# Lymphatus/caesium-clt

Hardware: AMD Instinct MI355X
Metric: megapixels/sec JPEG q=80 1920x1080 batch (higher is better)
Workload: dtype int32

## Files before the change

### caesium-clt_amd/csrc/k_trellis.hip

```cpp
#include <algorithm>
#include <atomic>
#include <cassert>
#include <utility>

#include "kernels.h"

namespace csh {

#define CSH_TR_CAP 16
#define CSH_TR_WGU uint32_t(CSH_TR_WG)
#define CSH_TR_SPILL (63 - CSH_TR_CAP)
#define CSH_TR_MAXWG 2048
size_t trellis_spill_words(uint32_t nslots) { return size_t(nslots) * CSH_TR_SPILL * 3u * CSH_TR_WGU; }

#ifdef CSH_EMUL
#define CSH_ANY(p) (p)
#define CSH_WAVE_OR(v) (v)
#define CSH_SPILL_LD(ptr) (*(ptr))
#define CSH_SPILL_ST(ptr, v) (*(ptr) = (v))
#else
#define CSH_ANY(p) (__ballot(p) != 0ull)
__device__ __forceinline__ static unsigned tr_wave_or(unsigned v) {
    const unsigned n = 32u - unsigned(__clz(v));
    unsigned r = 0;
    if (__ballot(n >= 8u)) r = 8u;
    if (__ballot(n >= r + 4u)) r += 4u;
    if (__ballot(n >= r + 2u)) r += 2u;
    if (__ballot(n >= r + 1u)) r += 1u;
    return r ? 1u << (r - 1u) : 0u;
}
#define CSH_WAVE_OR(v) tr_wave_or(v)
#define CSH_SPILL_LD(ptr) __builtin_nontemporal_load(ptr)
#define CSH_SPILL_ST(ptr, v) __builtin_nontemporal_store((v), (ptr))
#endif

using Oct8 = std::integer_sequence<int, 0, 1, 2, 3, 4, 5, 6, 7>;
static constexpr uint8_t kN2Z[64] = {0,  1,  5,  6,  14, 15, 27, 28, 2,  4,  7,  13, 16, 26, 29, 42, 3,  8,  12, 17, 25, 30,
                                     41, 43, 9,  11, 18, 24, 31, 40, 44, 53, 10, 19, 23, 32, 39, 45, 52, 54, 20, 22, 33, 38,
                                     46, 51, 55, 60, 21, 34, 37, 47, 50, 56, 59, 61, 35, 36, 48, 49, 57, 58, 62, 63};
template <int I>
__device__ __forceinline__ static int tr_half(const uint4 &v) {
    uint32_t w = (I / 2 == 0) ? v.x : (I / 2 == 1) ? v.y : (I / 2 == 2) ? v.z : v.w;
    return (I & 1) ? (int(w) >> 16) : (int(w << 16) >> 16);
}
template <int J, int... I>
__device__ __forceinline__ static void tr_unpack(int r[64], const uint4 &v, std::integer_sequence<int, I...>) { ((r[8 * J + I] = tr_half<I>(v)), ...); }
template <int... J>
__device__ __forceinline__ static void tr_load(const int16_t *__restrict__ blk, int r[64], std::integer_sequence<int, J...>) {
    const uint4 v[8] = {*reinterpret_cast<const uint4 *>(blk + CSH_RAW_OCT * J)...};
    (tr_unpack<J>(r, v[J], Oct8()), ...);
}
__device__ __forceinline__ static int tr_level(int x, int d, uint32_t mul, uint32_t sh) {
    const uint32_t a = uint32_t(x + (d >> 1)) << sh;
    return int(uint32_t((uint64_t(a & 0xFFFFFFu) * uint64_t(mul & 0xFFFFFFu)) >> 32));
}
__device__ __forceinline__ static int tr_bitlen(unsigned v) { return 32 - __clz(v); }
__device__ __forceinline__ static float tr_bits_f(uint32_t u) { float f; memcpy(&f, &u, 4); return f; }
__device__ __forceinline__ static uint32_t tr_f_bits(float f) { uint32_t u; memcpy(&u, &f, 4); return u; }

#define TRELLIS_LAMBDA_C1 0x1.ae89f995ad3adp+14
#define TRELLIS_LAMBDA_C2 0x1.6a09e667f3bcdp+16
#define TRELLIS_MAX_LEVEL 1023

struct TrLds {
    float (*A)[CSH_TR_WG];
    float (*Z)[CSH_TR_WG];
    uint32_t (*P)[CSH_TR_WG];
    const float *lenf;
    const float *runf;
    int lenEOB;
    const int32_t *q8;
    const uint32_t *qmul, *qsh;
    const float *lt;
    const float *rcp;
};

__device__ __forceinline__ static void trellis_stage(const TrellisCtx &c, uint32_t wi, float *s_lenf, float *s_runf, int *s_eob, int32_t *s_q8, uint32_t *s_qmul, uint32_t *s_qsh, float *s_lt, float *s_rcp) {
    const TrellisWork &w = c.work[wi];
    const ImgDesc &im = c.imgs[w.image];
    const DevQuant &Q = c.quant[im.qt_out[w.comp]];
    const int tid = int(threadIdx.x);
    const uint8_t *size = c.tables[w.table_ac].size;
    for (int i = tid; i < 16 * 11; i += CSH_TR_WG) {
        const int r = i / 11, sz = i % 11 + 1, l = sz <= 10 ? size[(r << 4) | sz] : 0;
        s_lenf[i] = l ? float(l + sz) : 1e38f;
    }
    if (tid < 4) s_runf[tid] = tid == 0 ? 0.0f : (size[0xF0] ? float(tid * int(size[0xF0])) : 1e38f);
    if (tid == 0) *s_eob = size[0x00];
    if (tid < 64) { s_q8[tid] = Q.div[tid]; s_qmul[tid] = Q.mul[tid]; s_qsh[tid] = Q.sh[tid]; s_lt[tid] = Q.lt[tid]; s_rcp[tid] = Q.rcp[tid]; }
}

__device__ __forceinline__ static void trellis_block(const TrellisCtx &c, uint32_t wi, uint32_t j, uint32_t wg_slot, const TrLds &L) {
    const TrellisWork &w = c.work[wi];
    const ImgDesc &im = c.imgs[w.image];
    const CompGeom g = im.out[w.comp];
    const int tid = int(threadIdx.x);
    const uint32_t slot = j * CSH_TR_WGU + uint32_t(tid);
    if (slot >= w.nunits) return;
    const uint32_t u = c.perm ? c.perm[w.unit_base + slot] : slot;
    const int by = int(u) / g.real_bw, b = by * g.bw + (int(u) - by * g.real_bw);
    uint32_t *sp = c.spill + size_t(wg_slot) * (CSH_TR_SPILL * 3u * CSH_TR_WGU) + uint32_t(tid);

    int r[64];
    tr_load(c.raw + raw_index(g.tile_base - c.raw_tile0, b), r, Oct8());
    CSH_SCHED_FENCE();
    float norm = 0.0f;
    CSH_UNROLL
    for (int n = 1; n < 64; n++) { const float vf = float(r[kN2Z[n]]); norm = norm + vf * vf; }
    norm = float(double(norm) / 63.0);
    const float lambda = float(TRELLIS_LAMBDA_C1 / (TRELLIS_LAMBDA_C2 + double(norm)));
    c.dcrec[w.unit_base + u] = (uint64_t(tr_f_bits(lambda)) << 32) | (uint32_t(r[0]) & 0xFFFFu);
    CSH_SCHED_FENCE();
    if (c.debug & 1u) return;

    uint32_t ne = 0;
    float Zrun = 0.0f;
    CSH_UNROLL
    for (int k = 1; k < 64; k++) {
        const int v = r[k], x = v < 0 ? -v : v;
        const float xf = float(x);
        int qv = int(tr_f_bits(__builtin_fmaf(xf, L.rcp[k], 12582912.0f)) & 0xFFFFu);
        qv = qv > TRELLIS_MAX_LEVEL ? TRELLIS_MAX_LEVEL : qv;
        if (qv) {
            const uint32_t P = uint32_t(x) | (uint32_t(k) << 15) | (uint32_t(qv) << 21) | (v < 0 ? 0x80000000u : 0u);
            if (ne < CSH_TR_CAP) { L.Z[ne][tid] = Zrun; L.P[ne][tid] = P; }
            else { CSH_SPILL_ST(sp + ((ne - CSH_TR_CAP) * 3u + 1u) * CSH_TR_WGU, tr_f_bits(Zrun)); CSH_SPILL_ST(sp + ((ne - CSH_TR_CAP) * 3u + 2u) * CSH_TR_WGU, P); }
            ne++;
        }
        Zrun = ((xf * xf) * lambda) * L.lt[k] + Zrun;
    }
    const float Z63 = Zrun;
    CSH_SCHED_FENCE();

    const float lenEOBf = float(L.lenEOB);
    if (c.debug & 2u) ne = 0;
    for (uint32_t t = 0; CSH_ANY(t < ne); t++) {
        const bool on = t < ne;
        float Zp; uint32_t P;
        if (t < CSH_TR_CAP) { Zp = L.Z[t][tid]; P = L.P[t][tid]; }
        else { Zp = tr_bits_f(CSH_SPILL_LD(sp + ((t - CSH_TR_CAP) * 3u + 1u) * CSH_TR_WGU)); P = CSH_SPILL_LD(sp + ((t - CSH_TR_CAP) * 3u + 2u) * CSH_TR_WGU); }
        if (!on) { Zp = 0.0f; P = 0u; }
        const int x = int(P & 0x7FFFu), kpos = int((P >> 15) & 63u), qval = int((P >> 21) & 1023u);
        const int q8 = L.q8[kpos];
        const float ltk = L.lt[kpos];
        const int ncand = on ? tr_bitlen(unsigned(qval)) : 0;
        const int ncmax = tr_bitlen(CSH_WAVE_OR(on ? unsigned(qval) : 0u));
        float dist[10];
        CSH_UNROLL
        for (int kc = 0; kc < 10; kc++) {
            dist[kc] = 1e38f;
            if (kc >= ncmax) continue;
            const int cand = kc < ncand - 1 ? (2 << kc) - 1 : qval;
            const int delta = __mul24(cand, q8) - x;
            dist[kc] = kc < ncand ? (float(__mul24(delta, delta)) * lambda) * ltk : 1e38f;
        }
        float bestc = 1e38f;
        uint32_t bestsel = 0;
        auto from = [&](int jj, int posj, float Aj, float Zj) {
            const int zr = kpos - 1 - posj;
            const float runf = L.runf[(zr >> 4) & 3];
            const float *lf = L.lenf + 11 * (zr & 15);
            const float tj = (Zp - Zj) + Aj;
            const uint32_t sel0 = uint32_t(jj + 1) << 4;
            CSH_UNROLL
            for (int kc = 0; kc < 10; kc++) {
                if (kc >= ncmax) break;
                const float cost = ((lf[kc] + runf) + dist[kc]) + tj;
                const bool better = cost < bestc;
                bestc = better ? cost : bestc;
                bestsel = better ? (sel0 | uint32_t(kc)) : bestsel;
            }
        };
        from(-1, 0, 0.0f, 0.0f);
        const int t_lds = int(t) < CSH_TR_CAP ? int(t) : CSH_TR_CAP;
        if (ncmax <= 4) {
            auto batch = [&](auto KCV) {
                constexpr int KC = decltype(KCV)::value;
                for (int j0 = 0; j0 < t_lds; j0 += 4) {
                    uint32_t Pj[4]; float Aj[4], Zj[4];
                    CSH_UNROLL
                    for (int i = 0; i < 4; i++) { const int r = j0 + i < CSH_TR_CAP ? j0 + i : CSH_TR_CAP - 1; Pj[i] = L.P[r][tid]; Aj[i] = L.A[r][tid]; Zj[i] = L.Z[r][tid]; }
                    float cost[4][KC];
                    CSH_UNROLL
                    for (int i = 0; i < 4; i++) {
                        const int zr = kpos - 1 - int((Pj[i] >> 15) & 63u);
                        const float runf = L.runf[(zr >> 4) & 3];
                        const float *lf = L.lenf + 11 * (zr & 15);
                        const float tj = j0 + i < t_lds ? (Zp - Zj[i]) + Aj[i] : 1e38f;
                        CSH_UNROLL
                        for (int kc = 0; kc < KC; kc++) cost[i][kc] = ((lf[kc] + runf) + dist[kc]) + tj;
                    }
                    CSH_UNROLL
                    for (int i = 0; i < 4; i++) {
                        CSH_UNROLL
                        for (int kc = 0; kc < KC; kc++) {
                            const bool better = cost[i][kc] < bestc;
                            bestc = better ? cost[i][kc] : bestc;
                            bestsel = better ? ((uint32_t(j0 + i + 1) << 4) | uint32_t(kc)) : bestsel;
                        }
                    }
                }
            };
            if (ncmax <= 1) batch(std::integral_constant<int, 1>());
            else if (ncmax == 2) batch(std::integral_constant<int, 2>());
            else if (ncmax == 3) batch(std::integral_constant<int, 3>());
            else batch(std::integral_constant<int, 4>());
        } else
            for (int jj = 0; jj < t_lds; jj++) from(jj, int((L.P[jj][tid] >> 15) & 63u), L.A[jj][tid], L.Z[jj][tid]);
        for (int jj = CSH_TR_CAP; jj < int(t); jj++) {
            const uint32_t *q = sp + (uint32_t(jj - CSH_TR_CAP) * 3u) * CSH_TR_WGU;
            from(jj, int((CSH_SPILL_LD(q + 2 * CSH_TR_WG) >> 15) & 63u), tr_bits_f(CSH_SPILL_LD(q)), tr_bits_f(CSH_SPILL_LD(q + CSH_TR_WG)));
        }
        if (on) {
            const int bk = int(bestsel & 15u);
            const uint32_t level = uint32_t(bk < ncand - 1 ? (2 << bk) - 1 : qval);
            const float Zi = (float(__mul24(x, x)) * lambda) * ltk + Zp;
            const uint32_t P2 = (bestsel >> 4) | ((level == uint32_t(qval) && qval < TRELLIS_MAX_LEVEL) ? 0x4000u : 0u) | (uint32_t(kpos) << 15) | (level << 21) | (P & 0x80000000u);
            if (t < CSH_TR_CAP) { L.A[t][tid] = bestc; L.Z[t][tid] = Zi; L.P[t][tid] = P2; }
            else { uint32_t *q = sp + ((t - CSH_TR_CAP) * 3u) * CSH_TR_WGU; CSH_SPILL_ST(q, tr_f_bits(bestc)); CSH_SPILL_ST(q + CSH_TR_WG, tr_f_bits(Zi)); CSH_SPILL_ST(q + 2 * CSH_TR_WG, P2); }
        }
    }

    float best = Z63 + lenEOBf;
    int last = -1;
    for (uint32_t e = 0; CSH_ANY(e < ne); e++) {
        float Ae, Ze; uint32_t Pe;
        if (e < CSH_TR_CAP) { Ae = L.A[e][tid]; Ze = L.Z[e][tid]; Pe = L.P[e][tid]; }
        else { const uint32_t *q = sp + ((e - CSH_TR_CAP) * 3u) * CSH_TR_WGU; Ae = tr_bits_f(CSH_SPILL_LD(q)); Ze = tr_bits_f(CSH_SPILL_LD(q + CSH_TR_WG)); Pe = CSH_SPILL_LD(q + 2 * CSH_TR_WG); }
        float cost = (Ae + Z63) - Ze;
        if (int((Pe >> 15) & 63u) < 63) cost = cost + lenEOBf;
        if (e < ne && cost < best) { best = cost; last = int(e); }
    }

    if (c.debug & 4u) return;
    uint64_t kept = 0;
    for (int e = last; CSH_ANY(e >= 0);) {
        if (e >= 0) {
            uint32_t Pe;
            if (e < CSH_TR_CAP) Pe = L.P[e][tid]; else Pe = CSH_SPILL_LD(sp + (uint32_t(e - CSH_TR_CAP) * 3u + 2u) * CSH_TR_WGU);
            kept |= 1ull << e;
            e = int(Pe & 63u) - 1;
        }
    }
    const bool to_tile = !(c.ac_lists && w.ac_lists);
    int16_t *dst = to_tile ? c.coef + coef_index(g.tile_base, b, 0) : nullptr;
    uint32_t *lst = nullptr;
    if (c.nz_pool && w.nzset != 0xFFFFFFFFu) {
        const NzSet &S = c.nzsets[w.nzset];
        const NzList &L0 = c.nzlists[S.list[0]];
        const uint32_t rec = L0.chunk0 + (u >> 8);
        if (c.nz_chunk_cnt[rec]) lst = c.nz_pool + L0.base + c.nz_chunk_off[rec] + c.blk_off[w.unit_base + u];
    }
    uint32_t room = ne;
    if (lst && c.blk_cnt) {
        room = c.blk_cnt[w.unit_base + u];
#ifdef CSH_EMUL
        if (room != ne) { fprintf(stderr, "k_trellis_ac: block %u of unit %u has %u list entries but %u levels\n", u, w.unit_base, room, ne); abort(); }
#endif
    }
    for (uint32_t e0 = 0; CSH_ANY(e0 < ne); e0 += 4) {
        uint32_t ent[4] = {0u, 0u, 0u, 0u};
        CSH_UNROLL
        for (uint32_t i = 0; i < 4; i++) {
            const uint32_t e = e0 + i;
            if (e < ne) {
                uint32_t Pe;
                if (e < CSH_TR_CAP) Pe = L.P[e][tid]; else Pe = CSH_SPILL_LD(sp + ((e - CSH_TR_CAP) * 3u + 2u) * CSH_TR_WGU);
                const int pos = int((Pe >> 15) & 63u), level = ((kept >> e) & 1ull) ? int((Pe >> 21) & 1023u) : 0;
                if (to_tile && !(((kept >> e) & 1ull) && (Pe & 0x4000u))) dst[coef_off(pos)] = int16_t((Pe >> 31) ? -level : level);
                ent[i] = uint32_t(pos) | ((Pe >> 31) ? 128u : 0u) | (uint32_t(level) << 8) | ((u & 255u) << 23);
            }
        }
        if (lst && e0 < ne && e0 < room) {
            if (e0 + 4 <= ne && e0 + 4 <= room) {
#ifdef CSH_EMUL
                memcpy(lst + e0, ent, 16);
#else
                typedef uint32_t tr_u32x4_a4 __attribute__((ext_vector_type(4), aligned(4)));
                tr_u32x4_a4 v; v.x = ent[0]; v.y = ent[1]; v.z = ent[2]; v.w = ent[3];
                *reinterpret_cast<tr_u32x4_a4 *>(lst + e0) = v;
#endif
            } else {
                CSH_UNROLL
                for (uint32_t i = 0; i < 4; i++) if (e0 + i < ne && e0 + i < room) lst[e0 + i] = ent[i];
            }
        }
    }
}

__global__ void __launch_bounds__(256) k_trellis_sort(TrellisCtx c) {
    CSH_SHARED uint32_t s_cnt[64];
    const TrellisWork w = c.work[blockIdx.x];
    const uint8_t *cnt = c.blk_cnt + w.unit_base;
    uint32_t *perm = c.perm + w.unit_base;
    CSH_PHASE_LOOP(4) {
        if (phase == 0) { if (threadIdx.x < 64) s_cnt[threadIdx.x] = 0; continue; }
        if (phase == 1) { for (uint32_t u = threadIdx.x; u < w.nunits; u += 256) atomicAdd(&s_cnt[cnt[u] & 63u], 1u); continue; }
        if (phase == 2) {
            if (threadIdx.x == 0) { uint32_t at = 0; for (int k = 63; k >= 0; k--) { const uint32_t n = s_cnt[k]; s_cnt[k] = at; at += n; } }
            continue;
        }
        for (uint32_t u = threadIdx.x; u < w.nunits; u += 256) perm[atomicAdd(&s_cnt[cnt[u] & 63u], 1u)] = u;
    }
}
void launch_trellis_sort(hipStream_t st, const TrellisCtx &c) { if (c.nwork && c.perm && c.blk_cnt) CSH_LAUNCH_PHASED(k_trellis_sort, 4, dim3(unsigned(c.nwork)), dim3(256), st, c); }

__global__ void __launch_bounds__(CSH_TR_WG) k_trellis_ac(TrellisCtx c) {
    CSH_SHARED float s_A[CSH_TR_CAP][CSH_TR_WG];
    CSH_SHARED float s_Z[CSH_TR_CAP][CSH_TR_WG];
    CSH_SHARED uint32_t s_P[CSH_TR_CAP][CSH_TR_WG];
    CSH_SHARED float s_lenf[16 * 11 + 16];
    CSH_SHARED float s_runf[4];
    CSH_SHARED int s_eob;
    CSH_SHARED int32_t s_q8[64];
    CSH_SHARED uint32_t s_qmul[64];
    CSH_SHARED uint32_t s_qsh[64];
    CSH_SHARED float s_lt[64];
    CSH_SHARED float s_rcp[64];
    TrLds L; L.A = s_A; L.Z = s_Z; L.P = s_P; L.lenf = s_lenf; L.runf = s_runf; L.q8 = s_q8; L.qmul = s_qmul; L.qsh = s_qsh; L.lt = s_lt; L.rcp = s_rcp;
#ifdef CSH_EMUL
    CSH_PHASE_LOOP(2) {
        const TrellisRun rn = c.runs[blockIdx.x];
        if (phase == 0) { trellis_stage(c, rn.work, s_lenf, s_runf, &s_eob, s_q8, s_qmul, s_qsh, s_lt, s_rcp); continue; }
        L.lenEOB = s_eob;
        for (uint32_t j = rn.j; j < rn.j + rn.n; j++) trellis_block(c, rn.work, j, 0u, L);
    }
#else
    CSH_SHARED uint32_t s_run;
    for (;;) {
        if (threadIdx.x == 0) s_run = atomicAdd(c.queue, 1u);
        __syncthreads();
        const uint32_t ri = s_run;
        if (ri >= c.nruns) break;
        const TrellisRun rn = c.runs[ri];
        trellis_stage(c, rn.work, s_lenf, s_runf, &s_eob, s_q8, s_qmul, s_qsh, s_lt, s_rcp);
        __syncthreads();
        L.lenEOB = s_eob;
        for (uint32_t j = rn.j; j < rn.j + rn.n; j++) trellis_block(c, rn.work, j, blockIdx.x, L);
        __syncthreads();
    }
#endif
}

__device__ static const uint8_t kStdDcLen[2][12] = {{2, 3, 3, 3, 3, 3, 4, 5, 6, 7, 8, 9}, {2, 2, 2, 3, 4, 5, 6, 7, 8, 9, 10, 11}};

__global__ void __launch_bounds__(64) k_trellis_dc(TrellisCtx c) {
    const uint32_t ri = blockIdx.x * blockDim.x + threadIdx.x;
    if (ri >= c.nrows) return;
    const uint32_t rr = c.rows[ri];
    const TrellisWork w = c.work[rr >> 16];
    const ImgDesc &im = c.imgs[w.image];
    const CompGeom g = im.out[w.comp];
    const DevQuant &Q = c.quant[im.qt_out[w.comp]];
    const int row = int(rr & 0xFFFFu);
    int ncand = (2 + 60 / int(Q.q[0])) | 1;
    ncand = ncand > 9 ? 9 : ncand;
    CSH_SHARED float s_costs[64][13];
    float *s_cost = s_costs[threadIdx.x & 63u];
    for (int i = 0; i < 12; i++) s_cost[i] = float(i + int(w.table_dc < 0 ? kStdDcLen[w.dc_cls ? 1 : 0][i] : c.tables[w.table_dc].size[i]));
    s_cost[12] = __builtin_inff();
    const int q = Q.div[0];
    const uint32_t qmul = Q.mul[0], qsh = Q.sh[0];
    const float lt0 = Q.lt[0];
    const int half = ncand / 2;
    int last_dc = 0;
    const int by1 = (row + 1) * g.v < g.real_bh ? (row + 1) * g.v : g.real_bh;
    for (int by = row * g.v; by < by1; by++) {
        float acc[9];
        int cprev[9];
        CSH_UNROLL
        for (int k = 0; k < 9; k++) { acc[k] = 0.0f; cprev[k] = 0; }
        int qprev = 0, sprev = 0;
        bool cprev_clamped = false;
        uint64_t rec_next = c.dcrec[w.unit_base + uint32_t(by * g.real_bw)];
        for (int bi = 0; bi < g.real_bw; bi++) {
            const uint32_t u = uint32_t(by * g.real_bw + bi);
            const uint64_t rec = rec_next;
            if (bi + 1 < g.real_bw) rec_next = c.dcrec[w.unit_base + u + 1u];
            const int raw0 = int(int16_t(uint16_t(rec & 0xFFFFu)));
            const float lambda_dc = tr_bits_f(uint32_t(rec >> 32)) * lt0;
            const int x = raw0 < 0 ? -raw0 : raw0;
            const int qval = tr_level(x, q, qmul, qsh);
            const int sgn = raw0 < 0 ? 1 : 0;
            const bool clamped = qval + half > TRELLIS_MAX_LEVEL;
            uint64_t bt = 0;
            float nacc[9];
            int ccur[9];
            float dist[9];
            CSH_UNROLL
            for (int k = 0; k < 9; k++) {
                int cand = qval - half + k;
                cand = cand > TRELLIS_MAX_LEVEL ? TRELLIS_MAX_LEVEL : cand;
                cand = cand < -TRELLIS_MAX_LEVEL ? -TRELLIS_MAX_LEVEL : cand;
                const int delta = k < ncand ? cand * q - x : 0;
                dist[k] = k < ncand ? float(delta * delta) * lambda_dc : __builtin_inff();
                ccur[k] = sgn ? -cand : cand;
            }
            if (bi == 0) {
                CSH_UNROLL
                for (int k = 0; k < 9; k++) { const int d = ccur[k] - last_dc, bits = tr_bitlen(unsigned(d < 0 ? -d : d)); nacc[k] = s_cost[bits] + dist[k]; }
            } else if (clamped || cprev_clamped) {
                CSH_UNROLL
                for (int k = 0; k < 9; k++) {
                    float bc = 0.0f;
                    uint32_t bl = 0;
                    CSH_UNROLL
                    for (int l = 0; l < 9; l++) {
                        const int d = ccur[k] - cprev[l], bits = tr_bitlen(unsigned(d < 0 ? -d : d));
                        const float cost = (s_cost[bits] + dist[k]) + acc[l];
                        if (l == 0 || cost < bc) { bc = cost; bl = uint32_t(l); }
                    }
                    nacc[k] = bc;
                    bt |= uint64_t(bl) << (4 * k);
                }
            } else {
                const bool same = sgn == sprev;
                const int base = same ? qval - qprev : qval + qprev - 2 * half;
                float cd[17];
                CSH_UNROLL
                for (int i = 0; i < 17; i++) { const int d = base + (i - 8); const int dd = same ? d : d + 8; cd[i] = s_cost[tr_bitlen(unsigned(dd < 0 ? -dd : dd))]; }
                CSH_UNROLL
                for (int k = 0; k < 9; k++) {
                    float bc = 0.0f;
                    uint32_t bl = 0;
                    CSH_UNROLL
                    for (int l = 0; l < 9; l++) {
                        const float cbits = same ? cd[k - l + 8] : cd[k + l];
                        const float cost = (cbits + dist[k]) + acc[l];
                        if (l == 0 || cost < bc) { bc = cost; bl = uint32_t(l); }
                    }
                    nacc[k] = bc;
                    bt |= uint64_t(bl) << (4 * k);
                }
            }
            CSH_UNROLL
            for (int k = 0; k < 9; k++) { acc[k] = nacc[k]; cprev[k] = ccur[k]; }
            qprev = qval; sprev = sgn; cprev_clamped = clamped;
            c.dcbt[w.unit_base + u] = bt | (uint64_t(uint32_t(qval)) << 36) | (uint64_t(raw0 < 0 ? 1u : 0u) << 47);
        }
        float bv = acc[0];
        uint32_t j = 0;
        CSH_UNROLL
        for (int i = 1; i < 9; i++) if (i < ncand && acc[i] < bv) { bv = acc[i]; j = uint32_t(i); }
        uint64_t bt_next = c.dcbt[w.unit_base + uint32_t(by * g.real_bw + g.real_bw - 1)];
        for (int bi = g.real_bw - 1; bi >= 0; bi--) {
            const uint64_t rec = bt_next;
            if (bi > 0) bt_next = c.dcbt[w.unit_base + uint32_t(by * g.real_bw + bi - 1)];
            int cand = int((rec >> 36) & 2047u) - half + int(j);
            cand = cand > TRELLIS_MAX_LEVEL ? TRELLIS_MAX_LEVEL : cand;
            cand = cand < -TRELLIS_MAX_LEVEL ? -TRELLIS_MAX_LEVEL : cand;
            cand = ((rec >> 47) & 1u) ? -cand : cand;
            c.coef[coef_index(g.tile_base, by * g.bw + bi, 0)] = int16_t(cand);
            if (bi == g.real_bw - 1) last_dc = cand;
            j = uint32_t((rec >> (4 * j)) & 15u);
        }
    }
}

#ifdef CSH_EMUL
uint32_t trellis_ac_slots() { return 1u; }
#else
uint32_t trellis_ac_slots() {
    static std::atomic<uint32_t> cached[64];
    int dev = 0;
    if (hipGetDevice(&dev) != hipSuccess) dev = 0;
    dev &= 63;
    uint32_t n = cached[dev].load(std::memory_order_relaxed);
    if (n) return n;
    int per_cu = 0, cus = 0;
    if (hipOccupancyMaxActiveBlocksPerMultiprocessor(&per_cu, k_trellis_ac, CSH_TR_WG, 0) != hipSuccess || per_cu < 1) per_cu = 1;
    if (hipDeviceGetAttribute(&cus, hipDeviceAttributeMultiprocessorCount, dev) != hipSuccess || cus < 1) cus = 1;
    n = uint32_t(per_cu) * uint32_t(cus);
    n = n < CSH_TR_MAXWG ? n : CSH_TR_MAXWG;
    cached[dev].store(n, std::memory_order_relaxed);
    return n;
}
#endif

void launch_trellis_ac(hipStream_t st, const TrellisCtx &c) {
    if (!c.nruns || !c.nslots) return;
#ifdef CSH_EMUL
    assert(c.nslots >= 1u);
    CSH_LAUNCH_PHASED(k_trellis_ac, 2, dim3(c.nruns), dim3(CSH_TR_WG), st, c);
#else
    const uint32_t nwg = std::min(std::min(c.nruns, c.nslots), trellis_ac_slots());
    CSH_LAUNCH(k_trellis_ac, dim3(nwg), dim3(CSH_TR_WG), st, c);
#endif
}
void launch_trellis_dc(hipStream_t st, const TrellisCtx &c) {
    if (c.nrows) CSH_LAUNCH(k_trellis_dc, dim3((c.nrows + 63) / 64), dim3(64), st, c);
}

}
```

Measured before the change: 49560.

## Restructure DC trellis to cut register pressure and batch backtrace loads

Reworks the DC trellis kernel so per-candidate levels and distortions are recomputed on the fly instead of kept in arrays. The rare clamped path now stages the accumulators and results in LDS behind non-unrolled loops. The common path walks candidates in a sign-dependent direction and reverses the result afterward. Backpointers are packed into two 32-bit halves, and the backtrace loads four records at a time to hide global-memory latency. The aim is lower VGPR use and shorter dependent load chains, at the cost of more LDS per thread and extra index arithmetic.

Result: no change. 49520, median of 3 (-0.1%).

```diff
diff --git a/caesium-clt_amd/csrc/k_trellis.hip b/caesium-clt_amd/csrc/k_trellis.hip
--- a/caesium-clt_amd/csrc/k_trellis.hip
+++ b/caesium-clt_amd/csrc/k_trellis.hip
@@ -344,6 +344,19 @@
 
 __device__ static const uint8_t kStdDcLen[2][12] = {{2, 3, 3, 3, 3, 3, 4, 5, 6, 7, 8, 9}, {2, 2, 2, 3, 4, 5, 6, 7, 8, 9, 10, 11}};
 
+#define CSH_DC_ACC 13
+#define CSH_DC_RES 22
+#define CSH_DC_COL 31
+#define CSH_DC_WALK 4
+
+__device__ __forceinline__ static int dc_level(int qv, int half, int k) {
+    int cand = qv - half + k;
+    cand = cand > TRELLIS_MAX_LEVEL ? TRELLIS_MAX_LEVEL : cand;
+    cand = cand < -TRELLIS_MAX_LEVEL ? -TRELLIS_MAX_LEVEL : cand;
+    return cand;
+}
+__device__ __forceinline__ static float dc_dist(int delta, bool real, float lambda_dc) { return real ? float(__mul24(delta, delta)) * lambda_dc : __builtin_inff(); }
+
 __global__ void __launch_bounds__(64) k_trellis_dc(TrellisCtx c) {
     const uint32_t ri = blockIdx.x * blockDim.x + threadIdx.x;
     if (ri >= c.nrows) return;
@@ -355,7 +368,7 @@
     const int row = int(rr & 0xFFFFu);
     int ncand = (2 + 60 / int(Q.q[0])) | 1;
     ncand = ncand > 9 ? 9 : ncand;
-    CSH_SHARED float s_costs[64][13];
+    CSH_SHARED float s_costs[64][CSH_DC_COL];
     float *s_cost = s_costs[threadIdx.x & 63u];
     for (int i = 0; i < 12; i++) s_cost[i] = float(i + int(w.table_dc < 0 ? kStdDcLen[w.dc_cls ? 1 : 0][i] : c.tables[w.table_dc].size[i]));
     s_cost[12] = __builtin_inff();
@@ -367,9 +380,8 @@
     const int by1 = (row + 1) * g.v < g.real_bh ? (row + 1) * g.v : g.real_bh;
     for (int by = row * g.v; by < by1; by++) {
         float acc[9];
-        int cprev[9];
         CSH_UNROLL
-        for (int k = 0; k < 9; k++) { acc[k] = 0.0f; cprev[k] = 0; }
+        for (int k = 0; k < 9; k++) acc[k] = 0.0f;
         int qprev = 0, sprev = 0;
         bool cprev_clamped = false;
         uint64_t rec_next = c.dcrec[w.unit_base + uint32_t(by * g.real_bw)];
@@ -383,76 +395,98 @@
             const int qval = tr_level(x, q, qmul, qsh);
             const int sgn = raw0 < 0 ? 1 : 0;
             const bool clamped = qval + half > TRELLIS_MAX_LEVEL;
-            uint64_t bt = 0;
+            uint32_t bt_lo = 0, bt_hi = 0;
             float nacc[9];
-            int ccur[9];
-            float dist[9];
-            CSH_UNROLL
-            for (int k = 0; k < 9; k++) {
-                int cand = qval - half + k;
-                cand = cand > TRELLIS_MAX_LEVEL ? TRELLIS_MAX_LEVEL : cand;
-                cand = cand < -TRELLIS_MAX_LEVEL ? -TRELLIS_MAX_LEVEL : cand;
-                const int delta = k < ncand ? cand * q - x : 0;
-                dist[k] = k < ncand ? float(delta * delta) * lambda_dc : __builtin_inff();
-                ccur[k] = sgn ? -cand : cand;
-            }
             if (bi == 0) {
                 CSH_UNROLL
-                for (int k = 0; k < 9; k++) { const int d = ccur[k] - last_dc, bits = tr_bitlen(unsigned(d < 0 ? -d : d)); nacc[k] = s_cost[bits] + dist[k]; }
+                for (int k = 0; k < 9; k++) {
+                    const int cand = dc_level(qval, half, k), ccur = sgn ? -cand : cand;
+                    const int d = ccur - last_dc, bits = tr_bitlen(unsigned(d < 0 ? -d : d));
+                    nacc[k] = s_cost[bits] + dc_dist(__mul24(cand, q) - x, k < ncand, lambda_dc);
+                }
             } else if (clamped || cprev_clamped) {
                 CSH_UNROLL
                 for (int k = 0; k < 9; k++) {
+                    s_cost[CSH_DC_ACC + k] = acc[k];
+                    s_cost[CSH_DC_RES + k] = dc_dist(__mul24(dc_level(qval, half, k), q) - x, k < ncand, lambda_dc);
+                }
+#pragma unroll 1
+                for (int k = 0; k < 9; k++) {
+                    const int cand = dc_level(qval, half, k), ccur = sgn ? -cand : cand;
+                    const float dk = s_cost[CSH_DC_RES + k];
+                    float bc = 0.0f;
+                    uint32_t bl = 0;
+#pragma unroll 1
+                    for (int l = 0; l < 9; l++) {
+                        const int pl = dc_level(qprev, half, l), d = ccur - (sprev ? -pl : pl), bits = tr_bitlen(unsigned(d < 0 ? -d : d));
+                        const float cost = (s_cost[bits] + dk) + s_cost[CSH_DC_ACC + l];
+                        if (l == 0 || cost < bc) { bc = cost; bl = uint32_t(l); }
+                    }
+                    s_cost[CSH_DC_RES + k] = bc;
+                    if (k < 8) bt_lo |= bl << (4 * k); else bt_hi = bl;
+                }
+                CSH_UNROLL
+                for (int k = 0; k < 9; k++) nacc[k] = s_cost[CSH_DC_RES + k];
+            } else {
+                const bool same = sgn == sprev;
+                const int step = same ? 1 : -1;
+                int dd = same ? qval - qprev - 8 : qval + qprev - 2 * half + 16;
+                float cd[17];
+                CSH_UNROLL
+                for (int i = 0; i < 17; i++) { cd[i] = s_cost[tr_bitlen(unsigned(dd < 0 ? -dd : dd))]; dd += step; }
+                int kk = same ? 0 : 8;
+                int delta = __mul24(qval - half + kk, q) - x;
+                const int dstep = same ? q : -q;
+                int sh = same ? 0 : 32;
+                const int shstep = same ? 4 : -4;
+                uint32_t bl0 = 0;
+                CSH_UNROLL
+                for (int j = 0; j < 9; j++) {
+                    const float dj = dc_dist(delta, kk < ncand, lambda_dc);
                     float bc = 0.0f;
                     uint32_t bl = 0;
                     CSH_UNROLL
                     for (int l = 0; l < 9; l++) {
-                        const int d = ccur[k] - cprev[l], bits = tr_bitlen(unsigned(d < 0 ? -d : d));
-                        const float cost = (s_cost[bits] + dist[k]) + acc[l];
+                        const float cost = (cd[j - l + 8] + dj) + acc[l];
                         if (l == 0 || cost < bc) { bc = cost; bl = uint32_t(l); }
                     }
-                    nacc[k] = bc;
-                    bt |= uint64_t(bl) << (4 * k);
+                    nacc[j] = bc;
+                    if (j == 0) bl0 = bl;
+                    else if (j < 8) bt_lo |= bl << sh;
+                    else { bt_lo |= same ? bl0 : bl; bt_hi = same ? bl : bl0; }
+                    kk += step; delta += dstep; sh += shstep;
                 }
-            } else {
-                const bool same = sgn == sprev;
-                const int base = same ? qval - qprev : qval + qprev - 2 * half;
-                float cd[17];
-                CSH_UNROLL
-                for (int i = 0; i < 17; i++) { const int d = base + (i - 8); const int dd = same ? d : d + 8; cd[i] = s_cost[tr_bitlen(unsigned(dd < 0 ? -dd : dd))]; }
-                CSH_UNROLL
-                for (int k = 0; k < 9; k++) {
-                    float bc = 0.0f;
-                    uint32_t bl = 0;
+                if (!same) {
                     CSH_UNROLL
-                    for (int l = 0; l < 9; l++) {
-                        const float cbits = same ? cd[k - l + 8] : cd[k + l];
-                        const float cost = (cbits + dist[k]) + acc[l];
-                        if (l == 0 || cost < bc) { bc = cost; bl = uint32_t(l); }
-                    }
-                    nacc[k] = bc;
-                    bt |= uint64_t(bl) << (4 * k);
+                    for (int j = 0; j < 4; j++) { const float t = nacc[j]; nacc[j] = nacc[8 - j]; nacc[8 - j] = t; }
                 }
             }
             CSH_UNROLL
-            for (int k = 0; k < 9; k++) { acc[k] = nacc[k]; cprev[k] = ccur[k]; }
+            for (int k = 0; k < 9; k++) acc[k] = nacc[k];
             qprev = qval; sprev = sgn; cprev_clamped = clamped;
-            c.dcbt[w.unit_base + u] = bt | (uint64_t(uint32_t(qval)) << 36) | (uint64_t(raw0 < 0 ? 1u : 0u) << 47);
+            c.dcbt[w.unit_base + u] = uint64_t(bt_lo) | (uint64_t(bt_hi | (uint32_t(qval) << 4) | (raw0 < 0 ? 1u << 15 : 0u)) << 32);
         }
         float bv = acc[0];
         uint32_t j = 0;
         CSH_UNROLL
         for (int i = 1; i < 9; i++) if (i < ncand && acc[i] < bv) { bv = acc[i]; j = uint32_t(i); }
-        uint64_t bt_next = c.dcbt[w.unit_base + uint32_t(by * g.real_bw + g.real_bw - 1)];
-        for (int bi = g.real_bw - 1; bi >= 0; bi--) {
-            const uint64_t rec = bt_next;
-            if (bi > 0) bt_next = c.dcbt[w.unit_base + uint32_t(by * g.real_bw + bi - 1)];
-            int cand = int((rec >> 36) & 2047u) - half + int(j);
-            cand = cand > TRELLIS_MAX_LEVEL ? TRELLIS_MAX_LEVEL : cand;
-            cand = cand < -TRELLIS_MAX_LEVEL ? -TRELLIS_MAX_LEVEL : cand;
-            cand = ((rec >> 47) & 1u) ? -cand : cand;
-            c.coef[coef_index(g.tile_base, by * g.bw + bi, 0)] = int16_t(cand);
-            if (bi == g.real_bw - 1) last_dc = cand;
-            j = uint32_t((rec >> (4 * j)) & 15u);
+        const uint64_t *bt_row = c.dcbt + w.unit_base + uint32_t(by * g.real_bw);
+        for (int b1 = g.real_bw - 1; b1 >= 0; b1 -= CSH_DC_WALK) {
+            uint64_t recs[CSH_DC_WALK];
+            CSH_UNROLL
+            for (int t = 0; t < CSH_DC_WALK; t++) recs[t] = bt_row[b1 - t > 0 ? b1 - t : 0];
+            int lv[CSH_DC_WALK];
+            CSH_UNROLL
+            for (int t = 0; t < CSH_DC_WALK; t++) {
+                const uint32_t lo = uint32_t(recs[t]), hi = uint32_t(recs[t] >> 32);
+                const int cand = dc_level(int((hi >> 4) & 2047u), half, int(j));
+                lv[t] = ((hi >> 15) & 1u) ? -cand : cand;
+                j = (j < 8u ? lo >> (4u * j) : hi) & 15u;
+            }
+            if (b1 == g.real_bw - 1) last_dc = lv[0];
+            CSH_UNROLL
+            for (int t = 0; t < CSH_DC_WALK; t++)
+                if (b1 - t >= 0) c.coef[coef_index(g.tile_base, by * g.bw + b1 - t, 0)] = int16_t(lv[t]);
         }
     }
 }
```
